# Mariachiar/Spatiotemporal-Deepfake-Detection-for-Live-Video-Calls

Hardware: AMD Instinct MI355X
Metric: clips/sec (32x3x224x224) (higher is better)
Workload: dtype bf16

## Files before the change

spatiotemporal-deepfake-detection-for-live-video-calls_amd/csrc/af_conv_ca.hip:

```cpp
#include "af_common.h"

namespace af {

struct CAArgs {
    const char* inb;
    const char* wc;
    const float* scale_c;
    const float* shift_c;
    const char* res;
    const char* in1;
    const char* w1;
    char* outx;
    const char* wa;
    const float* scale_a;
    const float* shift_a;
    char* outa;
    int T, HW, C, kslabs;
    int P, chunks, tiles;
#ifdef AF_STAMPS
    int dbg;
#endif
};
#ifdef AF_STAMPS
#define CA_DBG(bit) (a.dbg & (bit))
#else
#define CA_DBG(bit) false
#endif

template <int DT, bool DUAL, bool CWL>
__global__ __launch_bounds__(512, 2) void conv_ca_kernel(const CAArgs a) {
    typedef Elem<DT> E;
    static_assert(E::EPC == 8, "16-bit operands only");
    constexpr int BM = 256, TN = 4, TM = 2;
    constexpr int WROWS = 3 * 64;
    constexpr int WPIECES = WROWS / 64;
    constexpr int XPW = 4;
    static_assert(!(DUAL && CWL), "the projection form keeps both c weight sets in LDS anyway");
    constexpr int WBYTES = WROWS * 128;

    extern __shared__ uint4 smem[];
    const unsigned lds0 = (unsigned)(uintptr_t)(__attribute__((address_space(3))) char*)smem;
    const int tid = threadIdx.x, lane = tid & 63;
    const int wave = __builtin_amdgcn_readfirstlane(tid >> 6);
    const int frow = lane & 15, fg = lane >> 4;
    const int P = a.P;
    const int slot_bytes = (BM + P) * 128;
    constexpr int NIMG = DUAL ? 1 : 3;
    char* sm = reinterpret_cast<char*>(smem);
    char* img0 = sm + 2 * WBYTES;
    const int img_all = NIMG * slot_bytes + P * 128;
    char* cwl = img0 + img_all;
    char* wlds = cwl + (CWL ? 64 * 128 : 0);
    float* bnp = reinterpret_cast<float*>(wlds + (DUAL ? 2 * a.C * 128 : 0));
    const int wm = wave;

    for (int i = tid; i < a.C; i += 512) { bnp[i] = a.scale_c[i]; bnp[a.C + i] = a.shift_c[i]; }
    {
        uint4* z = reinterpret_cast<uint4*>(img0);
        for (int i = tid; i < img_all / 16; i += 512) z[i] = uint4{0u, 0u, 0u, 0u};
    }
    if (tid < 64) { bnp[2 * a.C + tid] = a.scale_a[tid]; bnp[2 * a.C + 64 + tid] = a.shift_a[tid]; }

    const int drow = lane >> 3, chunk = (lane & 7) ^ drow;
    const long long Kw = 3LL * a.C;
    const i32x4 wdesc = make_desc(a.wa);
    unsigned woff[WPIECES];
#pragma unroll
    for (int i = 0; i < WPIECES; ++i) {
        const int row = (wave + 8 * i) * 8 + drow, dt = row / 64, ch = row % 64;
        woff[i] = (unsigned)((ch * Kw + (long long)dt * a.C) * 2 + chunk * 16);
    }
    unsigned xoff[XPW];
    int xp[XPW];
#pragma unroll
    for (int i = 0; i < XPW; ++i) {
        const int row = (wave + 8 * i) * 8 + drow;
        const int t = row / P, p = row % P;
        xp[i] = p;
        xoff[i] = (unsigned)((((long long)t * a.HW + p) * a.C) * 2 + chunk * 16);
    }
    const long long clipx = (long long)a.T * a.HW * a.C * 2, clipb = (long long)a.T * a.HW * 64 * 2;

    const int my_tiles = (a.tiles - (int)blockIdx.x + (int)gridDim.x - 1) / (int)gridDim.x;
    const int total = my_tiles * a.kslabs;
    auto stage_tile = [&](int g) { return (int)blockIdx.x + (g / a.kslabs) * (int)gridDim.x; };
    auto issue_weights = [&](int g) {
        const unsigned base = lds0 + (g & 1) * WBYTES + wave * (8 * 128);
        const int soff = (g % a.kslabs) * 128;
#pragma unroll
        for (int i = 0; i < WPIECES; ++i) blds16_m0(woff[i], wdesc, soff, base + i * (64 * 128));
    };
    auto issue_image = [&](int g) {
        const int tile = stage_tile(g), n = tile / a.chunks, hw0 = (tile % a.chunks) * P;
        const i32x4 xdesc = make_desc(a.res + n * clipx + (long long)hw0 * a.C * 2);
        const unsigned base = lds0 + 2 * WBYTES + (g % 3) * slot_bytes + P * 128 + wave * (8 * 128);
        const int soff = (g % a.kslabs) * 128;
#pragma unroll
        for (int i = 0; i < XPW; ++i)
            blds16_nt_m0(hw0 + xp[i] < a.HW ? xoff[i] : kOutOfRange, xdesc, soff, base + i * (64 * 128));
    };
    const i32x4 cdesc = make_desc(a.wc);
    auto issue_cw = [&](int g) {
        blds16_m0((unsigned)((wave * 8 + drow) * 128 + chunk * 16), cdesc, (g % a.kslabs) * (64 * 128), lds0 + (unsigned)(cwl - sm) + wave * (8 * 128));
    };
    uint4 wcur[TN][2], bcur[TM][2], x0cur[TM][2];
    uint4 wnext[TN][2], bnext[TM][2], x0next[TM][2];
    auto load_wc = [&](uint4 (&dst)[TN][2], const char* wsrc, int kc) {
#pragma unroll
        for (int i = 0; i < TN; ++i)
#pragma unroll
            for (int kk = 0; kk < 2; ++kk)
                dst[i][kk] = gload16_uncounted(wsrc + ((long long)(kc * 64 + i * 16 + frow) * 64 + kk * 32 + fg * 8) * 2);
    };
    auto load_b = [&](uint4 (&dst)[TM][2], const char* bsrc, int tile) {
        const int n = tile / a.chunks, hw0 = (tile % a.chunks) * P;
        const char* bb = bsrc + n * clipb + (long long)hw0 * 64 * 2;
#pragma unroll
        for (int j = 0; j < TM; ++j) {
            const int r = wm * 32 + j * 16 + frow, t = r / P, p = r - t * P;
            const int pc = hw0 + p < a.HW ? p : 0;
#pragma unroll
            for (int kk = 0; kk < 2; ++kk) {
                if (CA_DBG(16)) {
                    const int r8 = wm * 32 + (2 * j + kk) * 8 + (lane >> 3), t8 = r8 / P, p8 = r8 - t8 * P;
                    dst[j][kk] = gload16_uncounted(bb + (((long long)t8 * a.HW + (hw0 + p8 < a.HW ? p8 : 0)) * 64 + (lane & 7) * 8) * 2);
                } else
                dst[j][kk] = gload16_uncounted(bb + (((long long)t * a.HW + pc) * 64 + kk * 32 + fg * 8) * 2);
            }
        }
    };

    f32x4 acc[TN][TM];
#pragma unroll
    for (int i = 0; i < TN; ++i)
#pragma unroll
        for (int j = 0; j < TM; ++j) acc[i][j] = f32x4{0.f, 0.f, 0.f, 0.f};

    if (total > 0) {
        if (!DUAL && !CWL) load_wc(wnext, a.wc, 0);
        load_b(bnext, a.inb, blockIdx.x);
        if (DUAL) {
            load_b(x0next, a.in1, blockIdx.x);
            const i32x4 d0 = make_desc(a.wc), d1 = make_desc(a.w1);
            const unsigned off = (unsigned)(drow * 128 + chunk * 16), base = lds0 + (unsigned)(wlds - sm) + wave * (8 * 128);
            for (int g = 0; g < a.C / 64; ++g) {
                blds16(off, d0, (g * 64 + wave * 8) * 128, base + g * (64 * 128));
                blds16(off, d1, (g * 64 + wave * 8) * 128, base + a.C * 128 + g * (64 * 128));
            }
        }
        issue_weights(0);
        if (CWL) issue_cw(0);
        if (!DUAL) {
            issue_image(0);
            if (total > 1) issue_image(1);
        }
    }
    __syncthreads();
    int c_tile = blockIdx.x, c_kc = 0;
    for (int q = 0; q < total; ++q) {
        if (q == 0) wait_vmcnt<0>();
        else if (!DUAL && q + 1 < total) wait_vmcnt<8>();
        else wait_vmcnt<4>();
        __builtin_amdgcn_s_barrier();
        if (CWL) {
#pragma unroll
            for (int i = 0; i < TN; ++i)
#pragma unroll
                for (int kk = 0; kk < 2; ++kk)
                    wcur[i][kk] = *reinterpret_cast<const uint4*>(cwl + (i * 16 + frow) * 128 + (((kk * 4 + fg) ^ (frow & 7)) << 4));
        } else if (!DUAL) {
#pragma unroll
            for (int i = 0; i < TN; ++i)
#pragma unroll
                for (int kk = 0; kk < 2; ++kk) {
                    u32x4 t = __builtin_bit_cast(u32x4, wnext[i][kk]);
                    asm volatile("" : "+v"(t));
                    wcur[i][kk] = __builtin_bit_cast(uint4, t);
                }
        }
        if (c_kc == 0) {
#pragma unroll
            for (int j = 0; j < TM; ++j)
#pragma unroll
                for (int kk = 0; kk < 2; ++kk) {
                    u32x4 t = __builtin_bit_cast(u32x4, bnext[j][kk]);
                    asm volatile("" : "+v"(t));
                    bcur[j][kk] = __builtin_bit_cast(uint4, t);
                    if (DUAL) {
                        u32x4 t0 = __builtin_bit_cast(u32x4, x0next[j][kk]);
                        asm volatile("" : "+v"(t0));
                        x0cur[j][kk] = __builtin_bit_cast(uint4, t0);
                    }
                }
        }
        const bool last = c_kc + 1 == a.kslabs;
        if (q + 1 < total) {
            if (!DUAL && !CWL && !CA_DBG(1)) load_wc(wnext, a.wc, last ? 0 : c_kc + 1);
            if (last && !CA_DBG(2)) {
                load_b(bnext, a.inb, c_tile + gridDim.x);
                if (DUAL) load_b(x0next, a.in1, c_tile + gridDim.x);
            }
            __builtin_amdgcn_sched_barrier(0);
            issue_weights(q + 1);
            if (!DUAL && !CWL && q + 2 < total) issue_image(q + 2);
        }
        __builtin_amdgcn_sched_barrier(0);
        const int n = c_tile / a.chunks, hw0 = (c_tile % a.chunks) * P;
        char* img = img0 + (DUAL ? 0 : q % 3) * slot_bytes;
        {
            f32x4 cc[TN][TM];
#pragma unroll
            for (int i = 0; i < TN; ++i)
#pragma unroll
                for (int j = 0; j < TM; ++j) cc[i][j] = f32x4{0.f, 0.f, 0.f, 0.f};
            u32x2 rcell[TN][TM];
            if (!DUAL) {
#pragma unroll
                for (int i = 0; i < TN; ++i)
#pragma unroll
                    for (int j = 0; j < TM; ++j) {
                        const int R = P + wm * 32 + j * 16 + frow;
                        rcell[i][j] = *reinterpret_cast<const u32x2*>(img + R * 128 + (((i * 2 + (fg >> 1)) ^ (frow & 7)) << 4) + (fg & 1) * 8);
                    }
            }
            f32x4 scv[2], sfv[2];
#pragma unroll
            for (int i = 0; i < 2; ++i) {
                scv[i] = *reinterpret_cast<const f32x4*>(bnp + c_kc * 64 + i * 16 + fg * 4);
                sfv[i] = *reinterpret_cast<const f32x4*>(bnp + a.C + c_kc * 64 + i * 16 + fg * 4);
            }
            __builtin_amdgcn_sched_barrier(0);
#pragma unroll
            for (int kk = 0; kk < 2; ++kk) {
                if (DUAL) {
                    const uint4* wl = reinterpret_cast<const uint4*>(wlds) + (c_kc * 64 + frow) * 8 + ((kk * 4 + fg) ^ (frow & 7));
#pragma unroll
                    for (int i = 0; i < TN; ++i) {
                        const uint4 w0 = wl[i * 16 * 8], w1 = wl[a.C * 8 + i * 16 * 8];
#pragma unroll
                        for (int j = 0; j < TM; ++j) {
                            Mma<DT>::run(w0, bcur[j][kk], cc[i][j]);
                            Mma<DT>::run(w1, x0cur[j][kk], cc[i][j]);
                        }
                    }
                } else {
#pragma unroll
                    for (int i = 0; i < TN; ++i)
#pragma unroll
                        for (int j = 0; j < TM; ++j) Mma<DT>::run(wcur[i][kk], bcur[j][kk], cc[i][j]);
                }
            }
            __builtin_amdgcn_sched_barrier(0);
#pragma unroll
            for (int i = 0; i < TN; ++i) {
                const f32x4 sc = scv[i & 1], sf = sfv[i & 1];
#pragma unroll
                for (int j = 0; j < TM; ++j) {
                    const int R = P + wm * 32 + j * 16 + frow;
                    char* cell = img + R * 128 + (((i * 2 + (fg >> 1)) ^ (frow & 7)) << 4) + (fg & 1) * 8;
                    f32x4 v = cc[i][j] * sc + sf;
                    if (!DUAL) v += Vec4<DT>::unpack(rcell[i][j]);
                    Vec4<DT>::store_relu(cell, v);
                }
                if (i + 2 < TN) {
                    scv[i & 1] = *reinterpret_cast<const f32x4*>(bnp + c_kc * 64 + (i + 2) * 16 + fg * 4);
                    sfv[i & 1] = *reinterpret_cast<const f32x4*>(bnp + a.C + c_kc * 64 + (i + 2) * 16 + fg * 4);
                }
                __builtin_amdgcn_sched_barrier(0);
            }
        }
        asm volatile("s_waitcnt lgkmcnt(0)" ::: "memory");
        __builtin_amdgcn_s_barrier();
        if (CWL && q + 1 < total) {
            if (!CA_DBG(1)) issue_cw(q + 1);
            if (q + 2 < total) issue_image(q + 2);
            __builtin_amdgcn_sched_barrier(0);
        }
        {
            char* ox = a.outx + ((long long)n * a.T * a.HW + hw0) * a.C * 2 + c_kc * 128;
#pragma unroll
            for (int it = 0; it < BM * 8 / 512; ++it) {
                const int row = (tid >> 3) + 64 * it, ck = tid & 7;
                const int t = row / P, p = row - t * P;
                const u32x4 o = *reinterpret_cast<const u32x4*>(img + (P + row) * 128 + ((ck ^ ((P + row) & 7)) << 4));
                if (hw0 + p < a.HW && !CA_DBG(8))
                    __builtin_nontemporal_store(o, reinterpret_cast<u32x4*>(ox + ((long long)t * a.HW + p) * a.C * 2 + ck * 16));
            }
        }
        const uint4* ws = smem + (q & 1) * (WBYTES / 16) + frow * 8;
        const uint4* xs = reinterpret_cast<const uint4*>(img) + (wm * 32 + frow) * 8;
        {
            uint4 af[2][TN], bf[2][TM];
            auto read_step = [&](uint4 (&fa)[TN], uint4 (&fb)[TM], int step) {
                const int dt = step >> 1, c = ((step & 1) * 4 + fg) ^ (frow & 7);
#pragma unroll
                for (int i = 0; i < TN; ++i) fa[i] = ws[(dt * 64 + i * 16) * 8 + c];
#pragma unroll
                for (int j = 0; j < TM; ++j) fb[j] = xs[(dt * P + j * 16) * 8 + c];
            };
            read_step(af[0], bf[0], 0);
#pragma unroll
            for (int step = 0; step < 6; ++step) {
                if (step + 1 < 6) read_step(af[(step + 1) & 1], bf[(step + 1) & 1], step + 1);
                __builtin_amdgcn_sched_barrier(0);
#pragma unroll
                for (int i = 0; i < TN; ++i)
#pragma unroll
                    for (int j = 0; j < TM; ++j) Mma<DT>::run(af[step & 1][i], bf[step & 1][j], acc[i][j]);
                __builtin_amdgcn_sched_barrier(0);
            }
        }
        if (!last) { ++c_kc; continue; }

#pragma unroll
        for (int j = 0; j < TM; ++j) {
            const int r = wm * 32 + j * 16 + frow;
            const int t = r / P, p = r - t * P;
            const long long pos = ((long long)n * a.T + t) * a.HW + hw0 + p;
#pragma unroll
            for (int ip = 0; ip < TN / 2; ++ip) {
                u32x2 half[2];
#pragma unroll
                for (int k = 0; k < 2; ++k) {
                    const int i = 2 * ip + k;
                    const f32x4 sc = *reinterpret_cast<const f32x4*>(bnp + 2 * a.C + i * 16 + fg * 4);
                    const f32x4 sf = *reinterpret_cast<const f32x4*>(bnp + 2 * a.C + 64 + i * 16 + fg * 4);
                    half[k] = Vec4<DT>::pack_relu(acc[i][j] * sc + sf);
                    acc[i][j] = f32x4{0.f, 0.f, 0.f, 0.f};
                }
                const u32x4 o = swap_pair16(half[0], half[1]);
                const int ch = (2 * ip + (fg & 1)) * 16 + (fg >> 1) * 8;
                if (hw0 + p < a.HW && !CA_DBG(4)) *reinterpret_cast<u32x4*>(a.outa + (pos * 64 + ch) * 2) = o;
            }
        }
        c_kc = 0; c_tile += gridDim.x;
    }
}

static long long conv_ca_lds_bytes(bool dual, int P, int C, bool cwl = false) {
    return 2LL * 3 * 64 * 128 + (dual ? (256LL + 2 * P) * 128 + 2LL * C * 128 : (3LL * (256 + P) + P) * 128 + (cwl ? 64 * 128 : 0)) + (2LL * C + 128) * 4;
}

template <int DT, bool DUAL, bool CWL>
static int launch_ca(const CAArgs& a, int blocks, hipStream_t stream) {
    const int lds = (int)conv_ca_lds_bytes(DUAL, a.P, a.C, CWL);
    if (lds > kLdsBudget) return set_error(AF_ERR_ARG, "conv_ca: %d bytes of LDS needed", lds);
    AF_SET_MAX_LDS((&conv_ca_kernel<DT, DUAL, CWL>), kLdsBudget, "conv_ca");
    hipLaunchKernelGGL((conv_ca_kernel<DT, DUAL, CWL>), dim3(blocks), dim3(512), lds, stream, a);
    AF_CHECK_LAUNCH("conv_ca_kernel");
    return AF_OK;
}

struct GeomCA { bool ok; int P, chunks, tiles; bool cwl; };
static GeomCA geom_ca(const af_conv_desc* dc, bool dual) {
    GeomCA g = {};
    if (dc->t != 16 && dc->t != 32) return g;
    const long long hw = (long long)dc->h * dc->w;
    if ((long long)dc->t * hw * dc->cout * 2 >= (1LL << 31)) return g;
    const int p = 256 / dc->t;
    if (conv_ca_lds_bytes(dual, p, dc->cout) > kLdsBudget) return g;
    if (hw % p != 0) return g;
    const long long tiles = (long long)dc->n * (hw / p);
    if (tiles < 4LL * device_cus() || tiles >= (1LL << 31)) return g;
    g.ok = true; g.P = p; g.chunks = (int)(hw / p); g.tiles = (int)tiles;
    g.cwl = !dual && conv_ca_lds_bytes(false, p, dc->cout, true) <= kLdsBudget;
    return g;
}

bool conv_ca_applies(const af_conv_desc* dc, const af_conv_desc* d1, const af_conv_desc* da) {
    if (!dc || !da) return false;
    if (d1) {
        if (d1->dtype != dc->dtype || d1->tpool || d1->kt != 1 || d1->kh != 1 || d1->kw != 1 || d1->st != 1 || d1->sh != 1 || d1->sw != 1) return false;
        if (d1->pt || d1->ph || d1->pw || d1->cin != 64 || d1->cout != dc->cout) return false;
        if (d1->n != dc->n || d1->t != dc->t || d1->h != dc->h || d1->w != dc->w) return false;
    }
    if (!dc || !da || dc->dtype == AF_F32 || da->dtype != dc->dtype || dc->tpool || da->tpool) return false;
    if (dc->kt != 1 || dc->kh != 1 || dc->kw != 1 || dc->st != 1 || dc->sh != 1 || dc->sw != 1 || dc->pt || dc->ph || dc->pw) return false;
    if (da->kt != 3 || da->kh != 1 || da->kw != 1 || da->st != 1 || da->sh != 1 || da->sw != 1 || da->pt != 1 || da->ph || da->pw) return false;
    if (dc->cin != 64 || da->cout != 64 || dc->cout != da->cin || dc->cout % 64 != 0 || dc->cout > 1024 || !dc->relu || !da->relu) return false;
    if (dc->n != da->n || dc->t != da->t || dc->h != da->h || dc->w != da->w) return false;
    return geom_ca(dc, d1 != nullptr).ok;
}

static int grid_ca(const GeomCA& g) {
    const int cus = device_cus();
    return g.tiles < cus ? g.tiles : cus;
}

bool conv_ca_work(const af_conv_desc* dc, const af_conv_desc* d1, const af_conv_desc* da, long long* tiles, int* workgroups, int* form,
                  int* pixels) {
    if (!conv_ca_applies(dc, d1, da)) return false;
    const GeomCA g = geom_ca(dc, d1 != nullptr);
    *tiles = g.tiles; *workgroups = grid_ca(g); *pixels = g.P;
    *form = d1 ? AF_CA_PROJECTION : g.cwl ? AF_CA_PLAIN_CWL : AF_CA_PLAIN;
    return true;
}

int conv_ca_run(const af_conv_desc* dc, const void* inb, const void* wc, const void* in1, const void* w1, const float* scale_c,
                const float* shift_c, const void* residual, void* outx, const af_conv_desc* da, const void* wa, const float* scale_a,
                const float* shift_a, void* outa, hipStream_t stream) {
    CAArgs a;
    a.inb = (const char*)inb; a.wc = (const char*)wc; a.scale_c = scale_c; a.shift_c = shift_c; a.res = (const char*)residual;
    a.in1 = (const char*)in1; a.w1 = (const char*)w1;
    a.outx = (char*)outx; a.wa = (const char*)wa; a.scale_a = scale_a; a.shift_a = shift_a; a.outa = (char*)outa;
    a.T = dc->t; a.HW = dc->h * dc->w; a.C = dc->cout; a.kslabs = dc->cout / 64;
    const GeomCA g = geom_ca(dc, in1 != nullptr);
    a.P = g.P; a.chunks = g.chunks; a.tiles = g.tiles;
    fill_dbg(a, "AF_CA_DBG");
    const int blocks = grid_ca(g);
    if (in1) return with_dtype16(dc->dtype, [&](auto dt) { return launch_ca<dt, true, false>(a, blocks, stream); });
    if (g.cwl)
        return with_dtype16(dc->dtype, [&](auto dt) { return launch_ca<dt, false, true>(a, blocks, stream); });
    return with_dtype16(dc->dtype, [&](auto dt) { return launch_ca<dt, false, false>(a, blocks, stream); });
}

}
```

Measured before the change: 3540.

## Interleave MFMA with BN updates and strength-reduce tile/address arithmetic in conv_ca

The per-tile index divisions and modulos are replaced with an incrementally advanced tile cursor, a rotating LDS slot counter and a running image pointer. Image-row store addresses and swizzled LDS offsets are precomputed once per thread, and the LDS reads for the output copy are batched before the stores. The matrix-multiply loop over output tiles is software-pipelined with the scale/shift update of the previous tile, using sched_group_barrier to interleave MFMA and VALU instructions. The bounds checks on image loads and output stores are dropped, which assumes the chunk size divides HW and could write out of range otherwise.

```diff
diff --git a/spatiotemporal-deepfake-detection-for-live-video-calls_amd/csrc/af_conv_ca.hip b/spatiotemporal-deepfake-detection-for-live-video-calls_amd/csrc/af_conv_ca.hip
--- a/spatiotemporal-deepfake-detection-for-live-video-calls_amd/csrc/af_conv_ca.hip
+++ b/spatiotemporal-deepfake-detection-for-live-video-calls_amd/csrc/af_conv_ca.hip
@@ -71,37 +71,54 @@
         woff[i] = (unsigned)((ch * Kw + (long long)dt * a.C) * 2 + chunk * 16);
     }
     unsigned xoff[XPW];
-    int xp[XPW];
 #pragma unroll
     for (int i = 0; i < XPW; ++i) {
         const int row = (wave + 8 * i) * 8 + drow;
         const int t = row / P, p = row % P;
-        xp[i] = p;
         xoff[i] = (unsigned)((((long long)t * a.HW + p) * a.C) * 2 + chunk * 16);
+    }
+    unsigned srow[BM * 8 / 512], simg[BM * 8 / 512];
+#pragma unroll
+    for (int it = 0; it < BM * 8 / 512; ++it) {
+        const int row = (tid >> 3) + 64 * it, ck = tid & 7;
+        const int t = row / P, p = row - t * P;
+        srow[it] = (unsigned)((((long long)t * a.HW + p) * a.C) * 2 + ck * 16);
+        simg[it] = (unsigned)((P + row) * 128 + ((ck ^ ((P + row) & 7)) << 4));
     }
     const long long clipx = (long long)a.T * a.HW * a.C * 2, clipb = (long long)a.T * a.HW * 64 * 2;
 
     const int my_tiles = (a.tiles - (int)blockIdx.x + (int)gridDim.x - 1) / (int)gridDim.x;
     const int total = my_tiles * a.kslabs;
-    auto stage_tile = [&](int g) { return (int)blockIdx.x + (g / a.kslabs) * (int)gridDim.x; };
-    auto issue_weights = [&](int g) {
+    const int gdiv = (int)gridDim.x / a.chunks, gmod = (int)gridDim.x % a.chunks;
+    struct TileCur { int n, ch; };
+    auto next_tile = [&](TileCur c) {
+        c.n += gdiv; c.ch += gmod;
+        if (c.ch >= a.chunks) { c.ch -= a.chunks; ++c.n; }
+        return c;
+    };
+    const TileCur tile0 = {(int)blockIdx.x / a.chunks, (int)blockIdx.x % a.chunks};
+    auto issue_weights = [&](int g, int kc) {
         const unsigned base = lds0 + (g & 1) * WBYTES + wave * (8 * 128);
-        const int soff = (g % a.kslabs) * 128;
+        const int soff = kc * 128;
 #pragma unroll
         for (int i = 0; i < WPIECES; ++i) blds16_m0(woff[i], wdesc, soff, base + i * (64 * 128));
     };
-    auto issue_image = [&](int g) {
-        const int tile = stage_tile(g), n = tile / a.chunks, hw0 = (tile % a.chunks) * P;
-        const i32x4 xdesc = make_desc(a.res + n * clipx + (long long)hw0 * a.C * 2);
-        const unsigned base = lds0 + 2 * WBYTES + (g % 3) * slot_bytes + P * 128 + wave * (8 * 128);
-        const int soff = (g % a.kslabs) * 128;
-#pragma unroll
-        for (int i = 0; i < XPW; ++i)
-            blds16_nt_m0(hw0 + xp[i] < a.HW ? xoff[i] : kOutOfRange, xdesc, soff, base + i * (64 * 128));
+    TileCur i_tile = tile0;
+    int i_kc = 0, i_slot = 0;
+    auto tile_bytes = [&](TileCur c) { return c.n * clipx + (long long)(c.ch * P) * a.C * 2; };
+    const char* i_res = a.res + tile_bytes(i_tile);
+    auto issue_image = [&]() {
+        const i32x4 xdesc = make_desc(i_res);
+        const unsigned base = lds0 + 2 * WBYTES + i_slot * slot_bytes + P * 128 + wave * (8 * 128);
+        const int soff = i_kc * 128;
+#pragma unroll
+        for (int i = 0; i < XPW; ++i) blds16_nt_m0(xoff[i], xdesc, soff, base + i * (64 * 128));
+        i_slot = i_slot == 2 ? 0 : i_slot + 1;
+        if (++i_kc == a.kslabs) { i_kc = 0; i_tile = next_tile(i_tile); i_res = a.res + tile_bytes(i_tile); }
     };
     const i32x4 cdesc = make_desc(a.wc);
-    auto issue_cw = [&](int g) {
-        blds16_m0((unsigned)((wave * 8 + drow) * 128 + chunk * 16), cdesc, (g % a.kslabs) * (64 * 128), lds0 + (unsigned)(cwl - sm) + wave * (8 * 128));
+    auto issue_cw = [&](int kc) {
+        blds16_m0((unsigned)((wave * 8 + drow) * 128 + chunk * 16), cdesc, kc * (64 * 128), lds0 + (unsigned)(cwl - sm) + wave * (8 * 128));
     };
     uint4 wcur[TN][2], bcur[TM][2], x0cur[TM][2];
     uint4 wnext[TN][2], bnext[TM][2], x0next[TM][2];
@@ -112,8 +129,8 @@
             for (int kk = 0; kk < 2; ++kk)
                 dst[i][kk] = gload16_uncounted(wsrc + ((long long)(kc * 64 + i * 16 + frow) * 64 + kk * 32 + fg * 8) * 2);
     };
-    auto load_b = [&](uint4 (&dst)[TM][2], const char* bsrc, int tile) {
-        const int n = tile / a.chunks, hw0 = (tile % a.chunks) * P;
+    auto load_b = [&](uint4 (&dst)[TM][2], const char* bsrc, TileCur tile) {
+        const int n = tile.n, hw0 = tile.ch * P;
         const char* bb = bsrc + n * clipb + (long long)hw0 * 64 * 2;
 #pragma unroll
         for (int j = 0; j < TM; ++j) {
@@ -138,9 +155,9 @@
 
     if (total > 0) {
         if (!DUAL && !CWL) load_wc(wnext, a.wc, 0);
-        load_b(bnext, a.inb, blockIdx.x);
+        load_b(bnext, a.inb, tile0);
         if (DUAL) {
-            load_b(x0next, a.in1, blockIdx.x);
+            load_b(x0next, a.in1, tile0);
             const i32x4 d0 = make_desc(a.wc), d1 = make_desc(a.w1);
             const unsigned off = (unsigned)(drow * 128 + chunk * 16), base = lds0 + (unsigned)(wlds - sm) + wave * (8 * 128);
             for (int g = 0; g < a.C / 64; ++g) {
@@ -148,15 +165,17 @@
                 blds16(off, d1, (g * 64 + wave * 8) * 128, base + a.C * 128 + g * (64 * 128));
             }
         }
-        issue_weights(0);
+        issue_weights(0, 0);
         if (CWL) issue_cw(0);
         if (!DUAL) {
-            issue_image(0);
-            if (total > 1) issue_image(1);
+            issue_image();
+            if (total > 1) issue_image();
         }
     }
     __syncthreads();
-    int c_tile = blockIdx.x, c_kc = 0;
+    TileCur c_tile = tile0;
+    int c_kc = 0, c_slot = 0;
+    char* c_ox = a.outx + tile_bytes(c_tile);
     for (int q = 0; q < total; ++q) {
         if (q == 0) wait_vmcnt<0>();
         else if (!DUAL && q + 1 < total) wait_vmcnt<8>();
@@ -194,19 +213,20 @@
                 }
         }
         const bool last = c_kc + 1 == a.kslabs;
+        const int n_kc = last ? 0 : c_kc + 1;
         if (q + 1 < total) {
             if (!DUAL && !CWL && !CA_DBG(1)) load_wc(wnext, a.wc, last ? 0 : c_kc + 1);
             if (last && !CA_DBG(2)) {
-                load_b(bnext, a.inb, c_tile + gridDim.x);
-                if (DUAL) load_b(x0next, a.in1, c_tile + gridDim.x);
+                load_b(bnext, a.inb, next_tile(c_tile));
+                if (DUAL) load_b(x0next, a.in1, next_tile(c_tile));
             }
             __builtin_amdgcn_sched_barrier(0);
-            issue_weights(q + 1);
-            if (!DUAL && !CWL && q + 2 < total) issue_image(q + 2);
+            issue_weights(q + 1, n_kc);
+            if (!DUAL && !CWL && q + 2 < total) issue_image();
         }
         __builtin_amdgcn_sched_barrier(0);
-        const int n = c_tile / a.chunks, hw0 = (c_tile % a.chunks) * P;
-        char* img = img0 + (DUAL ? 0 : q % 3) * slot_bytes;
+        const int n = c_tile.n, hw0 = c_tile.ch * P;
+        char* img = img0 + (DUAL ? 0 : c_slot) * slot_bytes;
         {
             f32x4 cc[TN][TM];
 #pragma unroll
@@ -230,29 +250,24 @@
                 sfv[i] = *reinterpret_cast<const f32x4*>(bnp + a.C + c_kc * 64 + i * 16 + fg * 4);
             }
             __builtin_amdgcn_sched_barrier(0);
-#pragma unroll
-            for (int kk = 0; kk < 2; ++kk) {
-                if (DUAL) {
-                    const uint4* wl = reinterpret_cast<const uint4*>(wlds) + (c_kc * 64 + frow) * 8 + ((kk * 4 + fg) ^ (frow & 7));
-#pragma unroll
-                    for (int i = 0; i < TN; ++i) {
+            auto mma_tile = [&](int i) {
+#pragma unroll
+                for (int kk = 0; kk < 2; ++kk) {
+                    if (DUAL) {
+                        const uint4* wl = reinterpret_cast<const uint4*>(wlds) + (c_kc * 64 + frow) * 8 + ((kk * 4 + fg) ^ (frow & 7));
                         const uint4 w0 = wl[i * 16 * 8], w1 = wl[a.C * 8 + i * 16 * 8];
 #pragma unroll
                         for (int j = 0; j < TM; ++j) {
                             Mma<DT>::run(w0, bcur[j][kk], cc[i][j]);
                             Mma<DT>::run(w1, x0cur[j][kk], cc[i][j]);
                         }
+                    } else {
+#pragma unroll
+                        for (int j = 0; j < TM; ++j) Mma<DT>::run(wcur[i][kk], bcur[j][kk], cc[i][j]);
                     }
-                } else {
-#pragma unroll
-                    for (int i = 0; i < TN; ++i)
-#pragma unroll
-                        for (int j = 0; j < TM; ++j) Mma<DT>::run(wcur[i][kk], bcur[j][kk], cc[i][j]);
-                }
-            }
-            __builtin_amdgcn_sched_barrier(0);
-#pragma unroll
-            for (int i = 0; i < TN; ++i) {
+                }
+            };
+            auto update_tile = [&](int i) {
                 const f32x4 sc = scv[i & 1], sf = sfv[i & 1];
 #pragma unroll
                 for (int j = 0; j < TM; ++j) {
@@ -266,26 +281,38 @@
                     scv[i & 1] = *reinterpret_cast<const f32x4*>(bnp + c_kc * 64 + (i + 2) * 16 + fg * 4);
                     sfv[i & 1] = *reinterpret_cast<const f32x4*>(bnp + a.C + c_kc * 64 + (i + 2) * 16 + fg * 4);
                 }
+            };
+            mma_tile(0);
+            __builtin_amdgcn_sched_barrier(0);
+#pragma unroll
+            for (int i = 1; i < TN; ++i) {
+                mma_tile(i);
+                update_tile(i - 1);
+#pragma unroll
+                for (int g = 0; g < (DUAL ? 8 : 4); ++g) {
+                    __builtin_amdgcn_sched_group_barrier(0x008, 1, 0);
+                    __builtin_amdgcn_sched_group_barrier(0x002, DUAL ? 3 : 7, 0);
+                }
                 __builtin_amdgcn_sched_barrier(0);
             }
+            update_tile(TN - 1);
+            __builtin_amdgcn_sched_barrier(0);
         }
         asm volatile("s_waitcnt lgkmcnt(0)" ::: "memory");
         __builtin_amdgcn_s_barrier();
         if (CWL && q + 1 < total) {
-            if (!CA_DBG(1)) issue_cw(q + 1);
-            if (q + 2 < total) issue_image(q + 2);
+            if (!CA_DBG(1)) issue_cw(n_kc);
+            if (q + 2 < total) issue_image();
             __builtin_amdgcn_sched_barrier(0);
         }
         {
-            char* ox = a.outx + ((long long)n * a.T * a.HW + hw0) * a.C * 2 + c_kc * 128;
-#pragma unroll
-            for (int it = 0; it < BM * 8 / 512; ++it) {
-                const int row = (tid >> 3) + 64 * it, ck = tid & 7;
-                const int t = row / P, p = row - t * P;
-                const u32x4 o = *reinterpret_cast<const u32x4*>(img + (P + row) * 128 + ((ck ^ ((P + row) & 7)) << 4));
-                if (hw0 + p < a.HW && !CA_DBG(8))
-                    __builtin_nontemporal_store(o, reinterpret_cast<u32x4*>(ox + ((long long)t * a.HW + p) * a.C * 2 + ck * 16));
-            }
+            char* ox = c_ox + c_kc * 128;
+            u32x4 o[BM * 8 / 512];
+#pragma unroll
+            for (int it = 0; it < BM * 8 / 512; ++it) o[it] = *reinterpret_cast<const u32x4*>(img + simg[it]);
+#pragma unroll
+            for (int it = 0; it < BM * 8 / 512; ++it)
+                if (!CA_DBG(8)) __builtin_nontemporal_store(o[it], reinterpret_cast<u32x4*>(ox + srow[it]));
         }
         const uint4* ws = smem + (q & 1) * (WBYTES / 16) + frow * 8;
         const uint4* xs = reinterpret_cast<const uint4*>(img) + (wm * 32 + frow) * 8;
@@ -310,6 +337,7 @@
                 __builtin_amdgcn_sched_barrier(0);
             }
         }
+        c_slot = c_slot == 2 ? 0 : c_slot + 1;
         if (!last) { ++c_kc; continue; }
 
 #pragma unroll
@@ -333,7 +361,7 @@
                 if (hw0 + p < a.HW && !CA_DBG(4)) *reinterpret_cast<u32x4*>(a.outa + (pos * 64 + ch) * 2) = o;
             }
         }
-        c_kc = 0; c_tile += gridDim.x;
+        c_kc = 0; c_tile = next_tile(c_tile); c_ox = a.outx + tile_bytes(c_tile);
     }
 }
 
```

Result: no change. 3550, median of 6 (+0.3%).
